# etri/bwa-mem-scale

Measured on AMD Instinct MI355X. Metric: Mreads/sec through the GPU hot path (seed -> chain -> extend -> dedup, reads and index resident), 150bp SE vs a synthetic genome of GRCh38 size, at 1 MI355X; % HBM roofline in roofline.frac, higher is better.
Workload: dtype int64 intervals / int16 DP (two columns per register; int32 for queries beyond 191 bases or scores beyond 2^14)

## Files before the change

bwa-mem-scale_amd/csrc/api.hip:

```cpp
#include <fcntl.h>
#include <sys/mman.h>
#include <sys/stat.h>
#include <unistd.h>

#include <algorithm>
#include <cstring>

#include "stage_state.h"

namespace bwams {

static Knobs g_knobs;
static std::once_flag g_knobs_once;
static int env_int(const char *name, int dflt) { const char *e = getenv(name); return e && *e ? atoi(e) : dflt; }
void knobs_reload() {
    Knobs k;
    { const char *vb = getenv("BWAMS_VERBOSE"); k.verbose = vb && *vb && *vb != '0'; }
    k.debug = env_int("BWAMS_DEBUG", 0);
    k.poison = env_int("BWAMS_POISON", 0);
    k.bwd_min_list = env_int("BWAMS_BWD_MIN_LIST", k.bwd_min_list); k.bwd_cols = env_int("BWAMS_BWD_COLS", k.bwd_cols);
    k.bwd_late_list = env_int("BWAMS_BWD_LATE_LIST", k.bwd_late_list);
    k.bwd_dry_min_list = env_int("BWAMS_BWD_DRY_MIN_LIST", k.bwd_dry_min_list); k.bwd_dry_cols = env_int("BWAMS_BWD_DRY_COLS", k.bwd_dry_cols);
    k.bwd_dry_late_list = env_int("BWAMS_BWD_DRY_LATE_LIST", k.bwd_dry_late_list);
    k.r3_beside = env_int("BWAMS_SEED_R3_BESIDE", 1);
    k.ext_max_rounds = env_int("BWAMS_EXT_MAX_ROUNDS", 0); k.ext_all_rounds = getenv("BWAMS_EXT_ALL_ROUNDS") != nullptr;
    k.ext_inplace = env_int("BWAMS_EXT_INPLACE", 1);
    k.dedup_seq = env_int("BWAMS_DEDUP_SEQ", 0) == 1;
    k.dedup_count = env_int("BWAMS_DEDUP_COUNT", 0) == 1;
    k.pair_count = env_int("BWAMS_PAIR_COUNT", 0) == 1;
    k.pair_drop_plan = getenv("BWAMS_PAIR_DROP_PLAN") != nullptr;
    k.trace_pair = env_int("BWAMS_TRACE_PAIR", 0);
    k.bsw_pk = env_int("BWAMS_BSW_PK", 1);
    k.chain_batch = env_int("BWAMS_CHAIN_BATCH", 1);
    k.chain_count = env_int("BWAMS_CHAIN_COUNT", 0) == 1;
    k.depth_combine = env_int("BWAMS_DEPTH_COMBINE", 1);
    k.pileup_tiled = env_int("BWAMS_PILEUP_TILED", 1);
    k.qc_lanes = env_int("BWAMS_QC_LANES", 1);
    k.recal_lds = env_int("BWAMS_RECAL_LDS", 1);
    k.ert_ticket = env_int("BWAMS_ERT_TICKET", 1); k.ert_grid = env_int("BWAMS_ERT_GRID", -1); k.ert_fat = env_int("BWAMS_ERT_FAT", 1);
    k.sa_dense = env_int("BWAMS_SA_DENSE", kSaDenseDefault);
    if (k.sa_dense != 0 && k.sa_dense != 1 && k.sa_dense != 2 && k.sa_dense != 4) k.sa_dense = kSaDenseDefault;
    { const char *mb = getenv("BWAMS_SA_DENSE_MAX_BYTES"); k.sa_dense_max_bytes = mb && *mb ? atoll(mb) : 0; }
    k.sort_narrow = env_int("BWAMS_SORT_NARROW", 1);
    g_knobs = k;
}
const Knobs &knobs() {
    std::call_once(g_knobs_once, knobs_reload);
    return g_knobs;
}

static thread_local std::string g_last_error;
void set_last_error(const std::string &s) { g_last_error = s; }

int check_device(int device) {
    int n = 0;
// ... 208 lines not shown
```

bwa-mem-scale_amd/csrc/api_extend.hip:

```cpp
#include <cstddef>

#include "stage_state.h"

using namespace bwams;

extern "C" {
static int ext_args(bwams_batch *b, StageState *s, const bwams_mem_opt_t *opt, ExtArgs *A) {
    const int64_t n1 = s->ch.nseq + 1;
    A->chains = s->ch.chains.p; A->n_chains = s->ch.n_chains; A->seeds = s->ch.seeds.p; A->n_seeds = s->ch.n_seeds;
    A->chain_off = s->ch.chain_off.as<int64_t>(); A->seed_off = s->ch.chain_off.as<int64_t>() + n1; A->enc = b->d_enc.p; A->cum = b->d_cum.p;
    A->nseq = s->ch.nseq; A->ref = b->idx->fmi.ref;
    int rc = dev_bns(b->idx, &A->bns);
    if (rc) return rc;
    A->opt = *opt; A->regs = s->ext.regs.p; A->srt = s->ext.srt.p; A->rmax = s->ext.rmax.as<int64_t>(); A->cnt = s->ext.cnt.as<int32_t>();
    A->ctr = b->d_ctr.p; A->state = s->ext.state.p; A->kreg = s->ext.kreg.p; A->cur = s->ext.cur.p; A->lim = s->ext.lim.p; A->sel_heavy = s->heavy.p;
    A->n_sel_heavy = &b->d_ctr.p->sel_heavy; A->sel_ticket = b->d_ctr.p->ext_sel_ticket; A->req_list = s->ext.req_list.p; A->rtask = nullptr;
    return BWAMS_OK;
}

static hipError_t ext_round_clear(bwams_batch *b) {
    DevCounters *c = b->d_ctr.p;
    return hipMemsetAsync(&c->ext_n_req, 0, (size_t)((char *)(c->ext_n_retry + 2) - (char *)&c->ext_n_req), b->stream);
}
static int ext_round_fetch(bwams_batch *b, int64_t *n_req, int64_t *n_rest, int64_t *n_l, int64_t *n_r) {
// ... 100 lines not shown
    if (n_right) *n_right = tot[3];
    produced(b, Product::built);
    return BWAMS_OK;
}

static int run_side(bwams_batch *b, StageState *s, const ExtArgs &A, int right, int64_t *n_retry_out) {
    hipStream_t st = b->stream;
    bwams_seqpair_t *pairs = right ? s->ext.rpairs.p : s->ext.lpairs.p;
    const bool ip = s->ext.tasks_inplace;
    const uint8_t *ref = ip ? A.ref : (right ? s->ext.rref.p : s->ext.lref.p);
    const uint8_t *qer = ip ? A.enc : (right ? s->ext.rqer.p : s->ext.lqer.p);
    const int64_t *src = ip ? (right ? s->ext.rsrc.as<int64_t>() : s->ext.lsrc.as<int64_t>()) : nullptr;
    const int dir = ip && !right ? -1 : 1;
    const int64_t n = right ? s->ext.n_right : s->ext.n_left;
    SwParams prm;
    sw_params(A.opt, right ? A.opt.pen_clip3 : A.opt.pen_clip5, &prm);
    const int qmax = b->max_read_len > 1 ? b->max_read_len : 1;
    if (n == 0) return BWAMS_OK;
    unsigned long long *d_nretry = &b->d_ctr.p->ext_n_retry[right], *h_nretry = &b->h_ctr.p->ext_n_retry[right];
    bwams_seqpair_t *rp = A.rtask ? s->ext.rpairs.p : nullptr;
    if (bsw_list_bytes(n) > b->sw.d_bsw_list.cap) BWAMS_HIP(hipStreamSynchronize(st));
    BWAMS_HIP(b->sw.d_bsw_list.ensure(bsw_list_bytes(n), bsw_list_bytes(n + n / 4 + 1024)));
    const bool verbose_bsw = knobs().verbose != 0;
    if (verbose_bsw) BWAMS_HIP(hipMemsetAsync(b->d_ctr.p->dbg + 40, 0, 8 * sizeof(unsigned long long), st));
    if (int lrc = launch_bsw(pairs, n, ref, qer, A.opt.w, prm, qmax, b->d_ctr.p, b->cu_count, st, b->sw.d_bsw_list.p, s->aux, s->fork, s->join, src, dir)) {
        set_last_error(lrc == -2 ? "banded SW: a query longer than ~18000 bases does not fit the LDS kernel" : "banded SW: stream fork/join failed");
        return lrc == -2 ? BWAMS_ERR_UNSUPPORTED : BWAMS_ERR_DEVICE;
    }
    launch_ext_post(A, right, pairs, n, A.opt.w, 0, s->ext.retry.p, d_nretry, rp, st);
    BWAMS_HIP(hipMemcpyAsync(h_nretry, d_nretry, sizeof(unsigned long long), hipMemcpyDeviceToHost, st));
    BWAMS_HIP(hipStreamSynchronize(st));
    if (verbose_bsw) {
        unsigned long long d[8];
        BWAMS_HIP(hipMemcpy(d, b->d_ctr.p->dbg + 40, sizeof d, hipMemcpyDeviceToHost));
        if (d[6])
            fprintf(stderr, "[run_side] bsw_pk_kernel, %s, %lld tasks: %llu waves, Mticks of wave-time %.2f, in the refill branch %.2f (%.1f %%), in the pass %.2f; "
                            "%llu refill events, %llu slots filled, %llu iterations\n",
                    right ? "right" : "left", (long long)n, d[6], d[0] / 1e6, d[1] / 1e6, 100. * (double)d[1] / (double)d[0], d[2] / 1e6, d[3], d[4], d[5]);
    }
    const unsigned long long nr = *h_nretry;
    if (nr) {
        if (launch_bsw(s->ext.retry.p, (int64_t)nr, ref, qer, A.opt.w << 1, prm, qmax, b->d_ctr.p, b->cu_count, st, b->sw.d_bsw_list.p, s->aux, s->fork, s->join, src, dir)) return BWAMS_ERR_DEVICE;
        launch_ext_post(A, right, s->ext.retry.p, (int64_t)nr, A.opt.w << 1, 1, nullptr, d_nretry, rp, st);
    }
    *n_retry_out += (int64_t)nr;
    return BWAMS_OK;
}

int bwams_extend_run(bwams_batch_t *b, const bwams_mem_opt_t *opt, int64_t *n_regs) {
    if (!has(b, Product::chains)) {
        set_last_error("bwams_extend_run: run bwams_chain_run (or bwams_chain_upload) first");
        return BWAMS_ERR_ARG;
    }
    if (!b->idx->fmi.ref) {
        set_last_error("bwams_extend_run: the index was opened without its .0123 reference");
        return BWAMS_ERR_ARG;
    }
    int rc = check_opt(opt, "bwams_extend_run");
    if (rc) return rc;
    int kMaxRounds = 6;
    if (knobs().ext_max_rounds > 0) kMaxRounds = knobs().ext_max_rounds;
    const bool adaptive_off = knobs().ext_all_rounds != 0;
    const bool inplace_on = knobs().ext_inplace != 0;
    StageState *s = b->stages;
    BWAMS_HIP(hipSetDevice(b->idx->device));
// ... 103 lines not shown
```

bwa-mem-scale_amd/csrc/api_sw.hip:

```cpp
#include "stage_state.h"

using namespace bwams;

extern "C" {

int bwams_bsw_upload(bwams_batch_t *b, const bwams_seqpair_t *pairs, int64_t n, const uint8_t *ref,
                     int64_t ref_bytes, const uint8_t *qer, int64_t qer_bytes) {
    if (!b || n < 0 || (n && (!pairs || !ref || !qer))) return BWAMS_ERR_ARG;
    BWAMS_HIP(hipSetDevice(b->idx->device));
    int qmax = 1, tmax = 1;
    for (int64_t i = 0; i < n; ++i) {
        const bwams_seqpair_t &p = pairs[i];
        if (p.len1 < 0 || p.len2 < 0 || p.idr < 0 || p.idq < 0 || (int64_t)p.idr + p.len1 > ref_bytes ||
            (int64_t)p.idq + p.len2 > qer_bytes) {
            set_last_error("bwams_bsw_upload: pair " + std::to_string(i) + " points outside the sequence buffers");
            return BWAMS_ERR_ARG;
        }
        if (p.len2 > qmax) qmax = p.len2;
        if (p.len1 > tmax) tmax = p.len1;
    }
    if (bsw_lds_waves(qmax) < 1) {
        set_last_error("bwams_bsw_upload: query of " + std::to_string(qmax) + " bases, longer than the LDS-resident kernel supports (18196)");
        return BWAMS_ERR_UNSUPPORTED;
    }
// ... 7 lines not shown
        BWAMS_HIP(hipMemcpyAsync(b->sw.d_qer.p, qer, (size_t)qer_bytes, hipMemcpyHostToDevice, b->stream));
        BWAMS_HIP(hipStreamSynchronize(b->stream));
    }
    b->sw.n_pairs = n;
    b->sw.max_qlen = qmax;
    b->sw.max_tlen = tmax;
    return BWAMS_OK;
}

int bwams_bsw_run(bwams_batch_t *b, int32_t w, const bwams_sw_opt_t *o) {
    if (!b || !o) return BWAMS_ERR_ARG;
    if (o->e_ins <= 0 || o->e_del <= 0) {
        set_last_error("bwams_bsw_run: gap extension penalties must be positive");
        return BWAMS_ERR_ARG;
    }
    BWAMS_HIP(hipSetDevice(b->idx->device));
    SwParams prm;
    sw_params(*o, &prm);
    BWAMS_HIP(hipMemsetAsync(&b->d_ctr.p->bsw_cells, 0, sizeof(unsigned long long), b->stream));
    const size_t list_bytes = b->sw.n_pairs > 0 ? bsw_list_bytes(b->sw.n_pairs) : 0;
    if (list_bytes > b->sw.d_bsw_list.cap) BWAMS_HIP(hipStreamSynchronize(b->stream));
    BWAMS_HIP(b->sw.d_bsw_list.ensure(list_bytes, bsw_list_bytes(b->sw.n_pairs + b->sw.n_pairs / 4 + 1024)));
    BWAMS_HIP(hipEventRecord(b->ev[b->kEvBswStart], b->stream));
    if (launch_bsw(b->sw.d_pairs.p, b->sw.n_pairs, b->sw.d_ref.p, b->sw.d_qer.p, w, prm, b->sw.max_qlen, b->d_ctr.p, b->cu_count, b->stream, b->sw.d_bsw_list.p)) {
        set_last_error("bwams_bsw_run: a query longer than ~18000 bases does not fit the LDS kernel");
        return BWAMS_ERR_UNSUPPORTED;
    }
    BWAMS_HIP(hipEventRecord(b->ev[b->kEvBswEnd], b->stream));
    BWAMS_HIP(hipGetLastError());
    return BWAMS_OK;
}

int bwams_bsw_fetch(bwams_batch_t *b, bwams_seqpair_t *pairs, int64_t n) {
    if (!b || n != b->sw.n_pairs) return BWAMS_ERR_ARG;
    BWAMS_HIP(hipSetDevice(b->idx->device));
    if (n) BWAMS_HIP(hipMemcpyAsync(pairs, b->sw.d_pairs.p, (size_t)n * sizeof(bwams_seqpair_t), hipMemcpyDeviceToHost, b->stream));
    BWAMS_HIP(hipStreamSynchronize(b->stream));
    return BWAMS_OK;
}

int bwams_bsw_extend(bwams_batch_t *b, bwams_seqpair_t *pairs, int64_t n, const uint8_t *ref, int64_t ref_bytes,
                     const uint8_t *qer, int64_t qer_bytes, int32_t w, const bwams_sw_opt_t *opt) {
    int rc = bwams_bsw_upload(b, pairs, n, ref, ref_bytes, qer, qer_bytes);
    if (rc) return rc;
    rc = bwams_bsw_run(b, w, opt);
    if (rc) return rc;
    return bwams_bsw_fetch(b, pairs, n);
// ... 42 lines not shown
```

bwa-mem-scale_amd/csrc/bsw_extend.hip:

```cpp
#include "common.h"
#include "wave_ops.h"

namespace bwams {

namespace {

constexpr int kWavesPerBlock = 4;
constexpr int kTaskChunk = 8;
constexpr size_t kBswLdsMax = 160 * 1024;

__host__ __device__ __forceinline__ size_t bsw_row_bytes(int qmax) {
    return (((size_t)(qmax + 1) * 8 + (size_t)qmax + 64 + 15) / 16) * 16;
}

__device__ __forceinline__ int wave_incl_prefix_max(int v, int lane) {
#pragma unroll
    for (int o = 1; o < 64; o <<= 1) {
        const int t = __shfl_up(v, o);
        if (lane >= o) v = max(v, t);
    }
    return v;
}

__global__ __launch_bounds__(kWavesPerBlock * 64) void bsw_kernel(
// ... 464 lines not shown
                ++i;
                fin = i >= tlen;
            }
            if (fin) {
                if (g == 0) {
                    bwams_seqpair_t *o = &pairs[cur];
                    o->score = mx; o->qle = max_j + 1; o->tle = max_i + 1; o->gtle = max_ie + 1; o->gscore = gscore; o->max_off = max_off;
                }
                alive = false;
            }
        }
    }
    for (int o = 32; o > 0; o >>= 1) cells += ((unsigned long long)__shfl_down((unsigned)(cells >> 32), o) << 32) | (unsigned)__shfl_down((unsigned)cells, o);
    if (lane == 0 && cells) atomicAdd(&ctr->bsw_cells, cells);
}


namespace pk {
__device__ __forceinline__ uint32_t add(uint32_t a, uint32_t b) { uint32_t d; asm("v_pk_add_u16 %0, %1, %2" : "=v"(d) : "v"(a), "v"(b)); return d; }
__device__ __forceinline__ uint32_t sub(uint32_t a, uint32_t b) { uint32_t d; asm("v_pk_sub_i16 %0, %1, %2" : "=v"(d) : "v"(a), "v"(b)); return d; }
__device__ __forceinline__ uint32_t max(uint32_t a, uint32_t b) { uint32_t d; asm("v_pk_max_i16 %0, %1, %2" : "=v"(d) : "v"(a), "v"(b)); return d; }
__device__ __forceinline__ uint32_t max0(uint32_t a) { uint32_t d; asm("v_pk_max_i16 %0, %1, 0" : "=v"(d) : "v"(a)); return d; }
__device__ __forceinline__ uint32_t mul(uint32_t a, uint32_t b) { uint32_t d; asm("v_pk_mul_lo_u16 %0, %1, %2" : "=v"(d) : "v"(a), "v"(b)); return d; }
__device__ __forceinline__ uint32_t adds(uint32_t a, uint32_t s) { uint32_t d; asm("v_pk_add_u16 %0, %1, %2" : "=v"(d) : "v"(a), "s"(s)); return d; }
__device__ __forceinline__ uint32_t subs(uint32_t a, uint32_t s) { uint32_t d; asm("v_pk_sub_i16 %0, %1, %2" : "=v"(d) : "v"(a), "s"(s)); return d; }
__device__ __forceinline__ uint32_t add2(uint32_t a) { uint32_t d; asm("v_pk_add_u16 %0, %1, 2 op_sel_hi:[1,0]" : "=v"(d) : "v"(a)); return d; }
__device__ __forceinline__ uint32_t min1(uint32_t a) { uint32_t d; asm("v_pk_min_u16 %0, %1, 1 op_sel_hi:[1,0]" : "=v"(d) : "v"(a)); return d; }
__device__ __forceinline__ uint32_t hi2(uint32_t a) { return __builtin_amdgcn_perm(a, a, 0x03020302u); }
__device__ __forceinline__ uint32_t lo2(uint32_t a) { return __builtin_amdgcn_perm(a, a, 0x01000100u); }
__device__ __forceinline__ uint32_t bfi(uint32_t mask, uint32_t a, uint32_t b) { uint32_t d; asm("v_bfi_b32 %0, %1, %2, %3" : "=v"(d) : "v"(mask), "v"(a), "v"(b)); return d; }
template <int CTRL> __device__ __forceinline__ int qdpp(int v) { return __builtin_amdgcn_update_dpp(0, v, CTRL, 0xF, 0xF, true); }
__device__ __forceinline__ int quad_all_max(int v) {
    int t = qdpp<0xB1>(v);
    v = v > t ? v : t;
    t = qdpp<0x4E>(v);
    return v > t ? v : t;
}
}

constexpr int kPkNeg = -16384;
#ifndef BWAMS_PK_WAVES
#define BWAMS_PK_WAVES 2
#endif
constexpr int kPkWaves = BWAMS_PK_WAVES;

__host__ __device__ __forceinline__ bool bsw_pk_eligible(const SwParams &prm) {
    for (int i = 0; i < 5; ++i)
        if (prm.mat[i * 5 + 4] != -1 || prm.mat[4 * 5 + i] != -1) return false;
    return prm.e_ins >= 0 && prm.e_ins <= 64 && prm.e_del >= 0 && prm.e_del <= 64 && prm.o_ins >= 0 && prm.o_ins + prm.e_ins < 8000 &&
           prm.o_del >= 0 && prm.o_del + prm.e_del < 8000;
}

__global__ __launch_bounds__(kPkWaves * 64) void bsw_pk_kernel(
    bwams_seqpair_t *__restrict__ pairs, const int32_t *__restrict__ list, const unsigned long long *n_list_p,
    const uint8_t *__restrict__ ref, const uint8_t *__restrict__ qer, int w0, SwParams prm, DevCounters *ctr, unsigned long long *head,
    int cols, const int64_t *__restrict__ src, int dir) {
    extern __shared__ __align__(16) uint32_t pk_lds[];
    constexpr int LPT = 4, TPW = 16;
    const int lane = threadIdx.x & 63, g = lane & (LPT - 1), q = lane / LPT;
    const int P = cols >> 1;
    uint32_t *const t_hp = pk_lds + 16 + (size_t)((threadIdx.x >> 6) * TPW + q) * (size_t)((5 * P) / 2 + 6);
    uint32_t *const t_ep = t_hp + P + 2;
    uint16_t *const t_sel = reinterpret_cast<uint16_t *>(t_ep + P + 2);
    uint16_t *const t_hp16 = reinterpret_cast<uint16_t *>(t_hp), *const t_ep16 = reinterpret_cast<uint16_t *>(t_ep);
    const int o_del = prm.o_del, e_del = prm.e_del, o_ins = prm.o_ins, e_ins = prm.e_ins;
    const int oe_del = o_del + e_del, oe_ins = o_ins + e_ins;
    uint2 *const pk_tab16 = reinterpret_cast<uint2 *>(pk_lds);
    if (threadIdx.x < 5) {
        const int t = threadIdx.x;
        pk_tab16[t] = make_uint2((uint32_t)(uint16_t)(int16_t)prm.mat[t * 5 + 0] | ((uint32_t)(uint16_t)(int16_t)prm.mat[t * 5 + 1] << 16),
                                 (uint32_t)(uint16_t)(int16_t)prm.mat[t * 5 + 2] | ((uint32_t)(uint16_t)(int16_t)prm.mat[t * 5 + 3] << 16));
    }
    __syncthreads();
    const uint32_t OEI = (uint32_t)oe_ins * 0x10001u, OED = (uint32_t)oe_del * 0x10001u, EDX = (uint32_t)e_del * 0x10001u;
    const uint32_t E1X = (uint32_t)e_ins * 0x10001u, E2X = (uint32_t)(2 * e_ins) * 0x10001u;
    const uint32_t NEGP = (uint32_t)(uint16_t)(int16_t)kPkNeg * 0x10001u;
    const int64_t n_list = (int64_t)*n_list_p;
    const unsigned long long kLeaders = 0x1111111111111111ull;
    int64_t pid = 0, pid_end = 0;
    bool exhausted = false;
    bool alive = false;
    int64_t pid0 = 0, s_qo = 0, s_to = 0;
    int s_cur = 0, s_tlen = 0, s_w = 0;
    uint32_t s_qh = 0u;
    int cur = 0, qlen = 0, tlen = 0, h0 = 0, w = 0, i = 0, beg = 0, end = 0;
    int mx = 0, max_i = -1, max_j = -1, max_ie = -1, gscore = -1, max_off = 0, tb_next = 4;
    const uint8_t *tr = ref;
    unsigned long long cells = 0;
    bool start_row = true, row = false;
    int base = 0, h1 = 0, key = -1, hlast = -1, c_max = kPkNeg, c_h = 0;
    int nz_last = 0, nz_first = 256;
    uint2 tt = make_uint2(0u, 0u);
#ifdef BWAMS_BSWDBG
    const unsigned long long T0 = __builtin_amdgcn_s_memtime();
    unsigned long long t_refill = 0, t_pass = 0, n_events = 0, n_filled = 0, n_iter = 0;
#endif

    for (;;) {
        const unsigned long long need_m = __ballot(!alive);
        if (need_m) {
#ifdef BWAMS_BSWDBG
            const unsigned long long Ta = __builtin_amdgcn_s_memtime();
#endif
            if (pid >= pid_end && !exhausted) {
                pid = (int64_t)wave_ticket(head, (unsigned long long)kQuadChunk);
                pid_end = pid + kQuadChunk < n_list ? pid + kQuadChunk : n_list;
                if (pid >= n_list) { exhausted = true; pid_end = pid; }
                pid0 = pid;
                if (lane < kQuadChunk && pid + lane < pid_end) {
                    s_cur = list[pid + lane];
                    const bwams_seqpair_t *sp = &pairs[s_cur];
                    const int l2 = sp->len2, hh0 = sp->h0;
                    s_tlen = sp->len1;
                    if (src) { const int64_t id = sp->id; s_qo = src[2 * id]; s_to = src[2 * id + 1]; }
                    else { s_qo = (int64_t)sp->idq; s_to = (int64_t)sp->idr; }
                    uint32_t tb = s_tlen > 0 ? (uint32_t)ref[s_to] : 4u;
                    tb = tb > 4u ? 4u : tb;
                    s_qh = (uint32_t)l2 | ((uint32_t)hh0 << 8) | (tb << 24);
// ... 1 lines not shown
                    int max_ins = (int)((double)(l2 * prm.max_sc + prm.end_bonus - o_ins) / e_ins + 1.);
                    max_ins = max_ins > 1 ? max_ins : 1;
                    ww = ww < max_ins ? ww : max_ins;
                    int max_del = (int)((double)(l2 * prm.max_sc + prm.end_bonus - o_del) / e_del + 1.);
                    max_del = max_del > 1 ? max_del : 1;
                    s_w = ww < max_del ? ww : max_del;
                }
            }
            const int avail = (int)(pid_end - pid);
            const int nq = __popcll(need_m & kLeaders);
            const int rank = __popcll(need_m & kLeaders & ((1ull << (q * LPT)) - 1ull));
            if (avail > 0) {
                const bool take = !alive && rank < avail;
                const int sk = take ? (int)(pid - pid0) + rank : 0;
                const int f_cur = __shfl(s_cur, sk), f_tlen = __shfl(s_tlen, sk), f_w = __shfl(s_w, sk);
                const uint32_t f_qh = (uint32_t)__shfl((int)s_qh, sk);
                const int64_t f_qo = shfl64(s_qo, sk), f_to = shfl64(s_to, sk);
                if (take) {
                    cur = f_cur; qlen = (int)(f_qh & 0xffu); h0 = (int)((f_qh >> 8) & 0x3fffu); tlen = f_tlen; w = f_w;
                    tr = ref + f_to;
                    start_row = true;
                    mx = h0; max_i = -1; max_j = -1; max_ie = -1; gscore = -1; max_off = 0;
                    beg = 0; end = qlen; i = 0;
                    alive = tlen > 0;
                    if (!alive && g == 0) {
                        bwams_seqpair_t *o = &pairs[cur];
                        o->score = mx; o->qle = 0; o->tle = 0; o->gtle = 0; o->gscore = -1; o->max_off = 0;
                    }
                    tb_next = (int)(f_qh >> 24);
                }
                for (unsigned long long fill_m = __ballot(take) & kLeaders; fill_m; fill_m &= fill_m - 1ull) {
                    const int sl = __ffsll((long long)fill_m) - 1;
                    const int f_qlen = __builtin_amdgcn_readlane(qlen, sl), f_h0 = __builtin_amdgcn_readlane(h0, sl);
                    const uint8_t *const f_q = qer + readlane64(f_qo, sl);
                    uint32_t *const f_hp = pk_lds + 16 + (size_t)((threadIdx.x >> 6) * TPW + (sl >> 2)) * (size_t)((5 * P) / 2 + 6);
                    uint32_t *const f_ep = f_hp + P + 2;
                    uint16_t *const f_sel = reinterpret_cast<uint16_t *>(f_ep + P + 2);
                    const int c0 = 4 * lane, p_last = f_qlen >> 1;
                    const bool full = c0 + 3 < f_qlen, edge = !full && c0 < f_qlen;
                    uint32_t v = 0u, b0 = 4u, b1 = 4u, b2 = 4u;
                    if (full) __builtin_memcpy(&v, dir > 0 ? f_q + c0 : f_q - c0 - 3, 4);
                    if (edge) {
                        const int last = f_qlen - 1;
                        b0 = f_q[c0 * dir];
                        b1 = f_q[(c0 + 1 < last ? c0 + 1 : last) * dir];
                        b2 = f_q[(c0 + 2 < last ? c0 + 2 : last) * dir];
// ... 31 lines not shown
            if (exhausted && !wave_any(alive)) break;
        }
#ifdef BWAMS_BSWDBG
        const unsigned long long Tb = __builtin_amdgcn_s_memtime();
#endif

        asm volatile("; BSW_PK_PASS_BEGIN");
        if (alive && start_row) {
            int tb = tb_next;
            tb = tb > 4 ? 4 : tb;
            if (i + 1 < tlen) tb_next = tr[(i + 1) * dir];
            tt = pk_tab16[tb];
            if (beg < i - w) beg = i - w;
            if (end > i + w + 1) end = i + w + 1;
            if (end > qlen) end = qlen;
            h1 = 0;
            if (beg == 0) {
                h1 = h0 - (o_del + e_del * (i + 1));
                h1 = h1 < 0 ? 0 : h1;
            }
            row = beg < end;
            key = -1; hlast = -1; nz_last = 0; nz_first = 256;
            c_max = kPkNeg; c_h = 0;
            base = beg & ~3;
            start_row = false;
        }
        {
            const bool in = alive && row;
            const int jb = base + g * 8;
            const bool inr = in && jb < cols;
            int lo = beg - jb, hi = end - jb;
            lo = lo < 0 ? 0 : (lo > 8 ? 8 : lo);
            hi = hi < 0 ? 0 : (hi > 8 ? 8 : hi);
            const uint32_t m8 = inr ? ((1u << hi) - 1u) & ~((1u << lo) - 1u) : 0u;
            const uint32_t m8x = m8 | (m8 << 15);
            const int pj = inr ? (jb >> 1) : 0;
            const uint2 hpa = *reinterpret_cast<const uint2 *>(t_hp + pj), hpb = *reinterpret_cast<const uint2 *>(t_hp + pj + 2);
            const uint2 epa = *reinterpret_cast<const uint2 *>(t_ep + pj), epb = *reinterpret_cast<const uint2 *>(t_ep + pj + 2);
            uint2 sl2;
            sl2.x = *reinterpret_cast<const uint32_t *>(t_sel + pj);
            sl2.y = *reinterpret_cast<const uint32_t *>(t_sel + pj + 2);
            const uint32_t hpv[4] = {hpa.x, hpa.y, hpb.x, hpb.y}, epv[4] = {epa.x, epa.y, epb.x, epb.y};
            const uint32_t slv[4] = {__builtin_amdgcn_perm(sl2.x, sl2.x, 0x01010000u) + 0x01000100u, __builtin_amdgcn_perm(sl2.x, sl2.x, 0x03030202u) + 0x01000100u,
                                     __builtin_amdgcn_perm(sl2.y, sl2.y, 0x01010000u) + 0x01000100u, __builtin_amdgcn_perm(sl2.y, sl2.y, 0x03030202u) + 0x01000100u};
            uint32_t AM[4], M[4], E[4], PX[4], JE[4], JP[4];
            JE[0] = (uint32_t)(jb * e_ins) * 0x10001u + ((uint32_t)e_ins << 16);
// ... 42 lines not shown
            for (int c = 0; c < 4; ++c) { F4[c] = pk::max(F4[c], Lexp); E2[c] = pk::subs(M[c], OED); }
#pragma unroll
            for (int c = 0; c < 4; ++c) { F4[c] = pk::sub(F4[c], JE[c]); T1[c] = pk::subs(E[c], EDX); ME[c] = pk::max(M[c], E[c]); }
#pragma unroll
            for (int c = 0; c < 4; ++c) { F4[c] = pk::adds(F4[c], E1X); E2[c] = pk::max(E2[c], T1[c]); }
#pragma unroll
            for (int c = 0; c < 4; ++c) { F4[c] = pk::max0(F4[c]); E2[c] = pk::max0(E2[c]); }
#pragma unroll
            for (int c = 0; c < 4; ++c) Hn[c] = pk::max(ME[c], F4[c]);
            const int h3 = (int)(Hn[3] >> 16);
            int hin = pk::qdpp<0x90>(h3);
            hin = g == 0 ? c_h : hin;
            uint32_t HL[4];
            HL[0] = __builtin_amdgcn_alignbit(Hn[0], (uint32_t)hin << 16, 16);
#pragma unroll
            for (int c = 1; c < 4; ++c) HL[c] = __builtin_amdgcn_alignbit(Hn[c], Hn[c - 1], 16);
            if (m8) {
                *reinterpret_cast<uint2 *>(t_hp + pj) = make_uint2(pk::bfi(AM[0], HL[0], hpv[0]), pk::bfi(AM[1], HL[1], hpv[1]));
                *reinterpret_cast<uint2 *>(t_hp + pj + 2) = make_uint2(pk::bfi(AM[2], HL[2], hpv[2]), pk::bfi(AM[3], HL[3], hpv[3]));
                *reinterpret_cast<uint2 *>(t_ep + pj) = make_uint2(pk::bfi(AM[0], E2[0], epv[0]), pk::bfi(AM[1], E2[1], epv[1]));
                *reinterpret_cast<uint2 *>(t_ep + pj + 2) = make_uint2(pk::bfi(AM[2], E2[2], epv[2]), pk::bfi(AM[3], E2[3], epv[3]));
            }
            int lkey = -1;
#pragma unroll
            for (int c = 0; c < 4; ++c) {
                const uint32_t ha = Hn[c] & AM[c];
                const int k0 = (int)__builtin_amdgcn_perm(ha, JP[c], 0x0c050400u), k1 = (int)__builtin_amdgcn_perm(ha, JP[c], 0x0c070602u);
                const int kk = k0 > k1 ? k0 : k1;
                lkey = lkey > kk ? lkey : kk;
            }
            {
                uint32_t NF[4];
#pragma unroll
                for (int c = 0; c < 4; ++c) NF[c] = (HL[c] | E2[c]) & AM[c];
#pragma unroll
                for (int c = 0; c < 4; ++c) NF[c] = pk::min1(NF[c]);
                const uint32_t nx = NF[0] | (NF[1] << 2) | (NF[2] << 4) | (NF[3] << 6);
                const int nl = (int)(((nx | (nx >> 15)) & 0xffu) << (8 * g));
                int nw = nl | pk::qdpp<0xB1>(nl);
                nw |= pk::qdpp<0x4E>(nw);
                const bool any = nw != 0;
                const int fc = any ? base + __builtin_ctz((unsigned)nw) : 256;
                nz_last = any ? base + 32 - __builtin_clz((unsigned)nw) : nz_last;
                nz_first = nz_first < fc ? nz_first : fc;
            }
            lkey = m8 ? lkey : -1;
            key = key > lkey ? key : lkey;
            {
                const int oe = hi - 1;
                if (m8 && jb + hi == end) {
                    uint32_t hv = Hn[0];
                    hv = (oe >> 1) == 1 ? Hn[1] : hv;
                    hv = (oe >> 1) == 2 ? Hn[2] : hv;
                    hv = (oe >> 1) == 3 ? Hn[3] : hv;
                    hlast = (int)((hv >> ((oe & 1) << 4)) & 0xffffu);
                }
            }
            if (in && base == (beg & ~3) && h1 != 0 && g == 0) t_hp16[beg] = (uint16_t)h1;
            const int pm = pk::qdpp<0xFF>(scan);
            const int ch = pk::qdpp<0xFF>(h3);
            const bool more = in && base + LPT * 8 < end;
            if (more) {
                c_max = c_max > pm ? c_max : pm;
                c_h = ch;
                base += LPT * 8;
            }
            const int rkey = pk::quad_all_max(key), rhl = pk::quad_all_max(hlast);
            int last_nz = nz_last - 1;
            int first_nz = nz_first;
            if (alive && !more) {
                if (row && h1 != 0) {
                    first_nz = first_nz < beg ? first_nz : beg;
                    last_nz = last_nz > beg ? last_nz : beg;
                }
                const int m = row ? rkey >> 8 : 0, mj = row ? (rkey & 0xff) - 1 : -1;
                const int h1f = row ? rhl : h1;
                if (g == 0) { t_hp16[end] = (uint16_t)h1f; t_ep16[end] = 0; }
                if (row) cells += (unsigned long long)(g == 0 ? end - beg : 0);
                const int j_exit = row ? end : beg;
                if (j_exit == qlen) {
                    max_ie = gscore > h1f ? max_ie : i;
                    gscore = gscore > h1f ? gscore : h1f;
                }
                const bool better = m > mx;
                const int di = i - max_i, dj = mj - max_j;
                const int zpen = di > dj ? (di - dj) * e_del : (dj - di) * e_ins;
                bool fin = m == 0 || (!better && prm.zdrop > 0 && mx - m - zpen > prm.zdrop);
                {
                    int d = mj - i;
                    d = d < 0 ? -d : d;
                    d = max_off > d ? max_off : d;
                    max_off = better ? d : max_off;
                    max_i = better ? i : max_i;
                    max_j = better ? mj : max_j;
                    mx = better ? m : mx;
                }
                {
                    const int nbeg = first_nz < end ? first_nz : end;
                    int jj = last_nz >= nbeg ? last_nz : nbeg - 1;
                    jj = h1f != 0 ? end : jj;
                    beg = nbeg;
                    end = jj + 2 < qlen ? jj + 2 : qlen;
                    ++i;
                    fin = fin || i >= tlen;
                }
                if (fin) {
                    if (g == 0) {
                        bwams_seqpair_t *o = &pairs[cur];
                        o->score = mx; o->qle = max_j + 1; o->tle = max_i + 1; o->gtle = max_ie + 1; o->gscore = gscore; o->max_off = max_off;
                    }
                    alive = false;
                }
                start_row = true;
            }
        }
        asm volatile("; BSW_PK_PASS_END");
#ifdef BWAMS_BSWDBG
        asm volatile("s_waitcnt vmcnt(0) lgkmcnt(0)" ::: "memory");
        t_pass += __builtin_amdgcn_s_memtime() - Tb;
        ++n_iter;
#endif
    }
#ifdef BWAMS_BSWDBG
    if (lane == 0) {
        unsigned long long *d = ctr->dbg + 40;
        atomicAdd(&d[0], __builtin_amdgcn_s_memtime() - T0); atomicAdd(&d[1], t_refill); atomicAdd(&d[2], t_pass);
        atomicAdd(&d[3], n_events); atomicAdd(&d[4], n_filled); atomicAdd(&d[5], n_iter); atomicAdd(&d[6], 1ull);
    }
#endif
    for (int o = 32; o > 0; o >>= 1) cells += ((unsigned long long)__shfl_down((unsigned)(cells >> 32), o) << 32) | (unsigned)__shfl_down((unsigned)cells, o);
    if (lane == 0 && cells) atomicAdd(&ctr->bsw_cells, cells);
}

__global__ void bsw_reset_kernel(DevCounters *ctr) {
    for (int i = 0; i < 4; ++i) ctr->bsw_head[i] = 0;
    for (int i = 0; i < kNumBswClass; ++i) ctr->bsw_cls_cnt[i] = ctr->bsw_cls_head[i] = 0;
}

}

int launch_bsw(bwams_seqpair_t *pairs, int64_t n, const uint8_t *ref, const uint8_t *qer, int w, const SwParams &prm, int qmax,
               DevCounters *ctr, int cu_count, hipStream_t st, int32_t *list, hipStream_t *aux, hipEvent_t fork, hipEvent_t *join,
               const int64_t *src, int dir) {
    bsw_reset_kernel<<<1, 1, 0, st>>>(ctr);
    if (n <= 0) return 0;
    bsw_classify_kernel<<<(unsigned)((n + 1023) / 1024), 1024, 0, st>>>(pairs, n, prm.max_sc, list, ctr->bsw_cls_cnt);
    int64_t blocks = (n + kWavesPerBlock - 1) / kWavesPerBlock;
    const int64_t maxb = (int64_t)cu_count * 8;
    if (blocks > maxb) blocks = maxb;
    hipStream_t q[5] = {st, st, st, st, st};
    const int n_aux = aux ? 4 : 0;
    if (n_aux) {
        if (hipEventRecord(fork, st) != hipSuccess) return -1;
        for (int c = 0; c < n_aux; ++c) {
            q[c + 1] = aux[c];
            if (hipStreamWaitEvent(q[c + 1], fork, 0) != hipSuccess) return -1;
        }
    }
    const unsigned B = (unsigned)blocks, T = kWavesPerBlock * 64;
    unsigned long long *cnt = ctr->bsw_cls_cnt, *hd = ctr->bsw_cls_head;
    auto pk_lds = [](int cols) { return (size_t)64 + (size_t)kPkWaves * 16 * ((size_t)(cols / 2) * 10 + 24); };
    {
        static std::mutex mu;
        static bool done[64] = {};
        int dev = 0;
        if (hipGetDevice(&dev) != hipSuccess) return -1;
        std::lock_guard<std::mutex> g(mu);
        if (dev < 0 || dev >= 64 || !done[dev]) {
            if (hipFuncSetAttribute(reinterpret_cast<const void *>(bsw_qwin_kernel<kBswLpt, kBswWin>), hipFuncAttributeMaxDynamicSharedMemorySize,
                                    (int)((size_t)kWavesPerBlock * (64 / kBswLpt) * 192 * 4)) != hipSuccess) return -1;
            if (hipFuncSetAttribute(reinterpret_cast<const void *>(bsw_pk_kernel), hipFuncAttributeMaxDynamicSharedMemorySize, (int)pk_lds(192)) != hipSuccess) return -1;
            if (dev >= 0 && dev < 64) done[dev] = true;
        }
    }
    const bool pk_env = knobs().bsw_pk != 0;
    if (pk_env && bsw_pk_eligible(prm)) {
        static const int kCols[5] = {32, 64, 96, 144, 192};
        const unsigned Bp = (unsigned)((int64_t)B * kWavesPerBlock / kPkWaves);
        for (int c = 4; c >= 0; --c)
            bsw_pk_kernel<<<Bp, kPkWaves * 64, pk_lds(kCols[c]), q[c]>>>(pairs, list + (int64_t)c * n, cnt + c, ref, qer, w, prm, ctr, hd + c, kCols[c], src, dir);
    } else {
    bsw_qwin_kernel<kBswLpt, kBswWin><<<B, T, (size_t)kWavesPerBlock * (64 / kBswLpt) * 192 * 4, q[4]>>>(pairs, list + 4 * n, cnt + 4, ref, qer, w, prm, ctr, hd + 4, 192, src, dir);
    bsw_qwin_kernel<kBswLpt, kBswWin><<<B, T, (size_t)kWavesPerBlock * (64 / kBswLpt) * 144 * 4, q[3]>>>(pairs, list + 3 * n, cnt + 3, ref, qer, w, prm, ctr, hd + 3, 144, src, dir);
    bsw_qwin_kernel<kBswLpt, kBswWin><<<B, T, (size_t)kWavesPerBlock * (64 / kBswLpt) * 96 * 4, q[2]>>>(pairs, list + 2 * n, cnt + 2, ref, qer, w, prm, ctr, hd + 2, 96, src, dir);
    bsw_qwin_kernel<kBswLpt, kBswWin><<<B, T, (size_t)kWavesPerBlock * (64 / kBswLpt) * 64 * 4, q[1]>>>(pairs, list + 1 * n, cnt + 1, ref, qer, w, prm, ctr, hd + 1, 64, src, dir);
    bsw_qwin_kernel<kBswLpt, kBswWin><<<B, T, (size_t)kWavesPerBlock * (64 / kBswLpt) * 32 * 4, q[0]>>>(pairs, list + 0 * n, cnt + 0, ref, qer, w, prm, ctr, hd + 0, 32, src, dir);
    }
    {
        const int waves = bsw_lds_waves(qmax);
        if (waves < 1) return -2;
        const size_t lds = bsw_row_bytes(qmax) * (size_t)waves;
        if (lds > 48 * 1024)
            (void)hipFuncSetAttribute(reinterpret_cast<const void *>(bsw_kernel),
                                      hipFuncAttributeMaxDynamicSharedMemorySize, (int)lds);
        int64_t lblocks = (n + waves - 1) / waves;
        const int64_t lcap = qmax > 16 * kQuadCpl[4] - 1 ? maxb : (int64_t)cu_count * 2;
        if (lblocks > lcap) lblocks = lcap;
        bsw_kernel<<<(unsigned)lblocks, waves * 64, lds, q[0]>>>(pairs, n, ref, qer, w, prm, qmax, -1, ctr, &ctr->bsw_head[3], list + 5 * n, cnt + 5, src, dir);
    }
    if (n_aux)
        for (int c = 0; c < n_aux; ++c) {
            if (hipEventRecord(join[c], q[c + 1]) != hipSuccess) return -1;
            if (hipStreamWaitEvent(st, join[c], 0) != hipSuccess) return -1;
// ... 12 lines not shown
```

bwa-mem-scale_amd/csrc/common.h:

```cpp
#pragma once

#include <atomic>
#include <cstdlib>
#include <hip/hip_runtime.h>
#include <mutex>
#include <shared_mutex>
#include <stdint.h>
#include <stdio.h>
#include <string>
#include <vector>

#include "../../include/bwams.h"
#include "stage_valid.h"

namespace bwams {

void set_last_error(const std::string &s);

constexpr int kSaDenseDefault = 1;
struct Knobs {
    int verbose = 0;
    int debug = 0;
    int poison = 0;
    int bwd_min_list = 40, bwd_cols = 24, bwd_late_list = 8;
    int bwd_dry_min_list = 24, bwd_dry_cols = 8, bwd_dry_late_list = 12;
    int r3_beside = 1;
    int ext_max_rounds = 0;
    int ext_all_rounds = 0;
    int ext_inplace = 1;
    int dedup_seq = 0;
    int dedup_count = 0;
    int pair_count = 0;
    int pair_drop_plan = 0;
    int trace_pair = 0;
    int bsw_pk = 1;
    int chain_count = 0;
    int chain_batch = 1;
    int ert_fat = 1;
    int depth_combine = 1;
    int pileup_tiled = 1;
    int qc_lanes = 1;
    int recal_lds = 1;
    int ert_grid = -1, ert_ticket = 1;
    int sa_dense = kSaDenseDefault;
    int64_t sa_dense_max_bytes = 0;
    int sort_narrow = 1;
};
const Knobs &knobs();
void knobs_reload();

int sa_dense_release(int device);

template <class T> static inline hipError_t dev_malloc(T **p, size_t bytes, bool may_yield = true) {
    const bool poison = knobs().poison != 0;
    hipError_t e = hipMalloc(reinterpret_cast<void **>(p), bytes);
    if (e == hipErrorOutOfMemory && may_yield) {
        int dev = 0;
        (void)hipGetLastError();
// ... 637 lines not shown
                       int out_on_device, int32_t flags, int64_t *n_out, bwams_deflate_stats_t *stats);

struct SwParams {
    int o_del, e_del, o_ins, e_ins, zdrop, end_bonus, max_sc;
    int8_t mat[25];
};

struct Round2Work {
    uint32_t rid;
    int32_t x;
    int32_t min_intv;
};

struct BwdItem {
    uint32_t rid;
    int32_t x;
    int32_t min_intv;
    int32_t num_prev;
    int64_t off;
};

int launch_bsw(bwams_seqpair_t *pairs, int64_t n, const uint8_t *ref, const uint8_t *qer, int w, const SwParams &prm, int qmax,
               DevCounters *ctr, int cu_count, hipStream_t st, int32_t *list, hipStream_t *aux = nullptr, hipEvent_t fork = nullptr,
               hipEvent_t *join = nullptr, const int64_t *src = nullptr, int dir = 1);
size_t bsw_list_bytes(int64_t n_tasks);
int bsw_lds_waves(int qmax);
void launch_emf_probe(const DevEmf &t, const uint8_t *enc, const int64_t *cum, int64_t nseq, uint32_t *out,
                      uint8_t *code, uint8_t *skip, DevCounters *ctr, hipStream_t st);
constexpr int KSW_XBYTE = 0x10000, KSW_XSTOP = 0x20000, KSW_XSUBO = 0x40000, KSW_XSTART = 0x80000;
constexpr int kKswMaxTarget = 20000;
int launch_ksw(const bwams_seqpair_t *pairs, int64_t n, const uint8_t *ref, const uint8_t *qer, const SwParams &prm,
                int pmax, int tmax, void *out, DevCounters *ctr, int cu_count, hipStream_t st);

struct SegMove { const char *src; char *dst; int64_t len; };
int segment_copy(const std::vector<SegMove> &moves, hipStream_t st);
int line_ends(const char *d_text, int64_t n_bytes, hipStream_t st, DevBuf<int64_t> *ends, int64_t *n_nl);

struct BnsMeta {
    int64_t l_pac = 0;
    std::vector<std::string> names, comments;
    std::vector<int64_t> ctg_off;
    std::vector<int32_t> ctg_len, ctg_ambs;
    std::vector<int64_t> hole_off;
    std::vector<int32_t> hole_len;
    std::vector<char> hole_amb;
    DevBuf<> d_pac;
};
// ... 194 lines not shown
```

Measured before the change: 11.95.

## Add early-termination bound to packed banded SW extension kernel

Adds a templated early-exit path to the packed int16 banded Smith-Waterman kernel. Each row computes an upper bound on the score any remaining cell could still reach (per-cell H/E plus the remaining query times the match score, and h1 plus the full query score). Once the band's tail is known and that bound cannot beat the current max or the global score, the task stops. It is on by default in the extension path (knob default -1) and adds per-row packed arithmetic plus a cross-lane max. It also pins waves_per_eu to 4, which may change register allocation and occupancy.

```diff
diff --git a/bwa-mem-scale_amd/csrc/api.hip b/bwa-mem-scale_amd/csrc/api.hip
--- a/bwa-mem-scale_amd/csrc/api.hip
+++ b/bwa-mem-scale_amd/csrc/api.hip
@@ -31,6 +31,7 @@
     k.pair_drop_plan = getenv("BWAMS_PAIR_DROP_PLAN") != nullptr;
     k.trace_pair = env_int("BWAMS_TRACE_PAIR", 0);
     k.bsw_pk = env_int("BWAMS_BSW_PK", 1);
+    k.bsw_early = env_int("BWAMS_BSW_EARLY", -1);
     k.chain_batch = env_int("BWAMS_CHAIN_BATCH", 1);
     k.chain_count = env_int("BWAMS_CHAIN_COUNT", 0) == 1;
     k.depth_combine = env_int("BWAMS_DEPTH_COMBINE", 1);
diff --git a/bwa-mem-scale_amd/csrc/api_extend.hip b/bwa-mem-scale_amd/csrc/api_extend.hip
--- a/bwa-mem-scale_amd/csrc/api_extend.hip
+++ b/bwa-mem-scale_amd/csrc/api_extend.hip
@@ -146,8 +146,9 @@
     if (bsw_list_bytes(n) > b->sw.d_bsw_list.cap) BWAMS_HIP(hipStreamSynchronize(st));
     BWAMS_HIP(b->sw.d_bsw_list.ensure(bsw_list_bytes(n), bsw_list_bytes(n + n / 4 + 1024)));
     const bool verbose_bsw = knobs().verbose != 0;
-    if (verbose_bsw) BWAMS_HIP(hipMemsetAsync(b->d_ctr.p->dbg + 40, 0, 8 * sizeof(unsigned long long), st));
-    if (int lrc = launch_bsw(pairs, n, ref, qer, A.opt.w, prm, qmax, b->d_ctr.p, b->cu_count, st, b->sw.d_bsw_list.p, s->aux, s->fork, s->join, src, dir)) {
+    const bool early = knobs().bsw_early != 0;
+    if (verbose_bsw) BWAMS_HIP(hipMemsetAsync(b->d_ctr.p->dbg + 40, 0, 10 * sizeof(unsigned long long), st));
+    if (int lrc = launch_bsw(pairs, n, ref, qer, A.opt.w, prm, qmax, b->d_ctr.p, b->cu_count, st, b->sw.d_bsw_list.p, s->aux, s->fork, s->join, src, dir, early)) {
         set_last_error(lrc == -2 ? "banded SW: a query longer than ~18000 bases does not fit the LDS kernel" : "banded SW: stream fork/join failed");
         return lrc == -2 ? BWAMS_ERR_UNSUPPORTED : BWAMS_ERR_DEVICE;
     }
@@ -155,16 +156,16 @@
     BWAMS_HIP(hipMemcpyAsync(h_nretry, d_nretry, sizeof(unsigned long long), hipMemcpyDeviceToHost, st));
     BWAMS_HIP(hipStreamSynchronize(st));
     if (verbose_bsw) {
-        unsigned long long d[8];
+        unsigned long long d[10];
         BWAMS_HIP(hipMemcpy(d, b->d_ctr.p->dbg + 40, sizeof d, hipMemcpyDeviceToHost));
         if (d[6])
             fprintf(stderr, "[run_side] bsw_pk_kernel, %s, %lld tasks: %llu waves, Mticks of wave-time %.2f, in the refill branch %.2f (%.1f %%), in the pass %.2f; "
-                            "%llu refill events, %llu slots filled, %llu iterations\n",
-                    right ? "right" : "left", (long long)n, d[6], d[0] / 1e6, d[1] / 1e6, 100. * (double)d[1] / (double)d[0], d[2] / 1e6, d[3], d[4], d[5]);
+                            "%llu refill events, %llu slots filled, %llu iterations, %llu rows, %llu tasks ended early\n",
+                    right ? "right" : "left", (long long)n, d[6], d[0] / 1e6, d[1] / 1e6, 100. * (double)d[1] / (double)d[0], d[2] / 1e6, d[3], d[4], d[5], d[7], d[8]);
     }
     const unsigned long long nr = *h_nretry;
     if (nr) {
-        if (launch_bsw(s->ext.retry.p, (int64_t)nr, ref, qer, A.opt.w << 1, prm, qmax, b->d_ctr.p, b->cu_count, st, b->sw.d_bsw_list.p, s->aux, s->fork, s->join, src, dir)) return BWAMS_ERR_DEVICE;
+        if (launch_bsw(s->ext.retry.p, (int64_t)nr, ref, qer, A.opt.w << 1, prm, qmax, b->d_ctr.p, b->cu_count, st, b->sw.d_bsw_list.p, s->aux, s->fork, s->join, src, dir, early)) return BWAMS_ERR_DEVICE;
         launch_ext_post(A, right, s->ext.retry.p, (int64_t)nr, A.opt.w << 1, 1, nullptr, d_nretry, rp, st);
     }
     *n_retry_out += (int64_t)nr;
diff --git a/bwa-mem-scale_amd/csrc/api_sw.hip b/bwa-mem-scale_amd/csrc/api_sw.hip
--- a/bwa-mem-scale_amd/csrc/api_sw.hip
+++ b/bwa-mem-scale_amd/csrc/api_sw.hip
@@ -53,7 +53,8 @@
     if (list_bytes > b->sw.d_bsw_list.cap) BWAMS_HIP(hipStreamSynchronize(b->stream));
     BWAMS_HIP(b->sw.d_bsw_list.ensure(list_bytes, bsw_list_bytes(b->sw.n_pairs + b->sw.n_pairs / 4 + 1024)));
     BWAMS_HIP(hipEventRecord(b->ev[b->kEvBswStart], b->stream));
-    if (launch_bsw(b->sw.d_pairs.p, b->sw.n_pairs, b->sw.d_ref.p, b->sw.d_qer.p, w, prm, b->sw.max_qlen, b->d_ctr.p, b->cu_count, b->stream, b->sw.d_bsw_list.p)) {
+    if (launch_bsw(b->sw.d_pairs.p, b->sw.n_pairs, b->sw.d_ref.p, b->sw.d_qer.p, w, prm, b->sw.max_qlen, b->d_ctr.p, b->cu_count, b->stream, b->sw.d_bsw_list.p,
+                   nullptr, nullptr, nullptr, nullptr, 1, knobs().bsw_early == 1)) {
         set_last_error("bwams_bsw_run: a query longer than ~18000 bases does not fit the LDS kernel");
         return BWAMS_ERR_UNSUPPORTED;
     }
diff --git a/bwa-mem-scale_amd/csrc/bsw_extend.hip b/bwa-mem-scale_amd/csrc/bsw_extend.hip
--- a/bwa-mem-scale_amd/csrc/bsw_extend.hip
+++ b/bwa-mem-scale_amd/csrc/bsw_extend.hip
@@ -510,6 +510,7 @@
 __device__ __forceinline__ uint32_t max(uint32_t a, uint32_t b) { uint32_t d; asm("v_pk_max_i16 %0, %1, %2" : "=v"(d) : "v"(a), "v"(b)); return d; }
 __device__ __forceinline__ uint32_t max0(uint32_t a) { uint32_t d; asm("v_pk_max_i16 %0, %1, 0" : "=v"(d) : "v"(a)); return d; }
 __device__ __forceinline__ uint32_t mul(uint32_t a, uint32_t b) { uint32_t d; asm("v_pk_mul_lo_u16 %0, %1, %2" : "=v"(d) : "v"(a), "v"(b)); return d; }
+__device__ __forceinline__ uint32_t mad(uint32_t a, uint32_t b, uint32_t c) { uint32_t d; asm("v_pk_mad_u16 %0, %1, %2, %3" : "=v"(d) : "v"(a), "v"(b), "v"(c)); return d; }
 __device__ __forceinline__ uint32_t adds(uint32_t a, uint32_t s) { uint32_t d; asm("v_pk_add_u16 %0, %1, %2" : "=v"(d) : "v"(a), "s"(s)); return d; }
 __device__ __forceinline__ uint32_t subs(uint32_t a, uint32_t s) { uint32_t d; asm("v_pk_sub_i16 %0, %1, %2" : "=v"(d) : "v"(a), "s"(s)); return d; }
 __device__ __forceinline__ uint32_t add2(uint32_t a) { uint32_t d; asm("v_pk_add_u16 %0, %1, 2 op_sel_hi:[1,0]" : "=v"(d) : "v"(a)); return d; }
@@ -530,6 +531,10 @@
 #ifndef BWAMS_PK_WAVES
 #define BWAMS_PK_WAVES 2
 #endif
+#ifndef BWAMS_BSW_EARLY_FORM
+#define BWAMS_BSW_EARLY_FORM 1
+#endif
+constexpr int kPkEarlyForm = BWAMS_BSW_EARLY_FORM;
 constexpr int kPkWaves = BWAMS_PK_WAVES;
 
 __host__ __device__ __forceinline__ bool bsw_pk_eligible(const SwParams &prm) {
@@ -539,7 +544,8 @@
            prm.o_del >= 0 && prm.o_del + prm.e_del < 8000;
 }
 
-__global__ __launch_bounds__(kPkWaves * 64) void bsw_pk_kernel(
+template <int EARLY>
+__global__ __launch_bounds__(kPkWaves * 64) __attribute__((amdgpu_waves_per_eu(4, 4))) void bsw_pk_kernel(
     bwams_seqpair_t *__restrict__ pairs, const int32_t *__restrict__ list, const unsigned long long *n_list_p,
     const uint8_t *__restrict__ ref, const uint8_t *__restrict__ qer, int w0, SwParams prm, DevCounters *ctr, unsigned long long *head,
     int cols, const int64_t *__restrict__ src, int dir) {
@@ -579,9 +585,11 @@
     int base = 0, h1 = 0, key = -1, hlast = -1, c_max = kPkNeg, c_h = 0;
     int nz_last = 0, nz_first = 256;
     uint2 tt = make_uint2(0u, 0u);
+    int zr = 0;
+    uint32_t pot = 0u;
 #ifdef BWAMS_BSWDBG
     const unsigned long long T0 = __builtin_amdgcn_s_memtime();
-    unsigned long long t_refill = 0, t_pass = 0, n_events = 0, n_filled = 0, n_iter = 0;
+    unsigned long long t_refill = 0, t_pass = 0, n_events = 0, n_filled = 0, n_iter = 0, n_rows = 0, n_rule = 0;
 #endif
 
     for (;;) {
@@ -629,6 +637,7 @@
                     start_row = true;
                     mx = h0; max_i = -1; max_j = -1; max_ie = -1; gscore = -1; max_off = 0;
                     beg = 0; end = qlen; i = 0;
+                    if constexpr (EARLY != 0) zr = qlen;
                     alive = tlen > 0;
                     if (!alive && g == 0) {
                         bwams_seqpair_t *o = &pairs[cur];
@@ -706,6 +715,7 @@
             row = beg < end;
             key = -1; hlast = -1; nz_last = 0; nz_first = 256;
             c_max = kPkNeg; c_h = 0;
+            if constexpr (EARLY != 0) pot = 0u;
             base = beg & ~3;
             start_row = false;
         }
@@ -794,6 +804,20 @@
                 *reinterpret_cast<uint2 *>(t_ep + pj + 2) = make_uint2(pk::bfi(AM[2], E2[2], epv[2]), pk::bfi(AM[3], E2[3], epv[3]));
             }
             int lkey = -1;
+            if constexpr (EARLY != 0) {
+                const uint32_t A2X = (uint32_t)(2 * prm.max_sc) * 0x10001u;
+                uint32_t RM[4], X[4], T[4];
+                RM[0] = pk::lo2((uint32_t)__mul24(qlen - 1 - jb, prm.max_sc)) - ((uint32_t)prm.max_sc << 16);
+#pragma unroll
+                for (int c = 1; c < 4; ++c) RM[c] = pk::subs(RM[c - 1], A2X);
+#pragma unroll
+                for (int c = 0; c < 4; ++c) X[c] = pk::max(Hn[c] & AM[c], E2[c]);
+#pragma unroll
+                for (int c = 0; c < 4; ++c) T[c] = pk::min1(X[c]);
+#pragma unroll
+                for (int c = 0; c < 4; ++c) X[c] = pk::mad(T[c], RM[c], X[c]);
+                pot = pk::max(pot, pk::max(pk::max(X[0], X[1]), pk::max(X[2], X[3])));
+            }
 #pragma unroll
             for (int c = 0; c < 4; ++c) {
                 const uint32_t ha = Hn[c] & AM[c];
@@ -838,6 +862,11 @@
                 base += LPT * 8;
             }
             const int rkey = pk::quad_all_max(key), rhl = pk::quad_all_max(hlast);
+            int rpot = 0;
+            if constexpr (EARLY != 0) {
+                const int a = (int)(pot & 0xffffu), b = (int)(pot >> 16);
+                rpot = pk::quad_all_max(a > b ? a : b);
+            }
             int last_nz = nz_last - 1;
             int first_nz = nz_first;
             if (alive && !more) {
@@ -871,6 +900,21 @@
                     const int nbeg = first_nz < end ? first_nz : end;
                     int jj = last_nz >= nbeg ? last_nz : nbeg - 1;
                     jj = h1f != 0 ? end : jj;
+                    if constexpr (EARLY != 0) {
+                        int P = h1 + __mul24(qlen, prm.max_sc);
+                        P = h1 > 0 ? P : 0;
+                        P = P > rpot ? P : rpot;
+                        const bool tail_known = end >= zr;
+                        zr = tail_known ? jj : zr;
+                        const bool ends = tail_known && P <= mx && P < gscore && (EARLY == 1 || (i & 3) == 3);
+#ifdef BWAMS_BSWDBG
+                        if (g == 0 && ends && !fin && i + 1 < tlen) ++n_rule;
+#endif
+                        fin = fin || ends;
+                    }
+#ifdef BWAMS_BSWDBG
+                    if (g == 0) ++n_rows;
+#endif
                     beg = nbeg;
                     end = jj + 2 < qlen ? jj + 2 : qlen;
                     ++i;
@@ -899,6 +943,7 @@
         atomicAdd(&d[0], __builtin_amdgcn_s_memtime() - T0); atomicAdd(&d[1], t_refill); atomicAdd(&d[2], t_pass);
         atomicAdd(&d[3], n_events); atomicAdd(&d[4], n_filled); atomicAdd(&d[5], n_iter); atomicAdd(&d[6], 1ull);
     }
+    if (g == 0 && n_rows) { atomicAdd(&ctr->dbg[47], n_rows); atomicAdd(&ctr->dbg[48], n_rule); }
 #endif
     for (int o = 32; o > 0; o >>= 1) cells += ((unsigned long long)__shfl_down((unsigned)(cells >> 32), o) << 32) | (unsigned)__shfl_down((unsigned)cells, o);
     if (lane == 0 && cells) atomicAdd(&ctr->bsw_cells, cells);
@@ -913,7 +958,7 @@
 
 int launch_bsw(bwams_seqpair_t *pairs, int64_t n, const uint8_t *ref, const uint8_t *qer, int w, const SwParams &prm, int qmax,
                DevCounters *ctr, int cu_count, hipStream_t st, int32_t *list, hipStream_t *aux, hipEvent_t fork, hipEvent_t *join,
-               const int64_t *src, int dir) {
+               const int64_t *src, int dir, bool early) {
     bsw_reset_kernel<<<1, 1, 0, st>>>(ctr);
     if (n <= 0) return 0;
     bsw_classify_kernel<<<(unsigned)((n + 1023) / 1024), 1024, 0, st>>>(pairs, n, prm.max_sc, list, ctr->bsw_cls_cnt);
@@ -941,7 +986,8 @@
         if (dev < 0 || dev >= 64 || !done[dev]) {
             if (hipFuncSetAttribute(reinterpret_cast<const void *>(bsw_qwin_kernel<kBswLpt, kBswWin>), hipFuncAttributeMaxDynamicSharedMemorySize,
                                     (int)((size_t)kWavesPerBlock * (64 / kBswLpt) * 192 * 4)) != hipSuccess) return -1;
-            if (hipFuncSetAttribute(reinterpret_cast<const void *>(bsw_pk_kernel), hipFuncAttributeMaxDynamicSharedMemorySize, (int)pk_lds(192)) != hipSuccess) return -1;
+            if (hipFuncSetAttribute(reinterpret_cast<const void *>(bsw_pk_kernel<0>), hipFuncAttributeMaxDynamicSharedMemorySize, (int)pk_lds(192)) != hipSuccess) return -1;
+            if (hipFuncSetAttribute(reinterpret_cast<const void *>(bsw_pk_kernel<kPkEarlyForm>), hipFuncAttributeMaxDynamicSharedMemorySize, (int)pk_lds(192)) != hipSuccess) return -1;
             if (dev >= 0 && dev < 64) done[dev] = true;
         }
     }
@@ -949,8 +995,9 @@
     if (pk_env && bsw_pk_eligible(prm)) {
         static const int kCols[5] = {32, 64, 96, 144, 192};
         const unsigned Bp = (unsigned)((int64_t)B * kWavesPerBlock / kPkWaves);
+        auto *const kern = early && prm.max_sc > 0 ? bsw_pk_kernel<kPkEarlyForm> : bsw_pk_kernel<0>;
         for (int c = 4; c >= 0; --c)
-            bsw_pk_kernel<<<Bp, kPkWaves * 64, pk_lds(kCols[c]), q[c]>>>(pairs, list + (int64_t)c * n, cnt + c, ref, qer, w, prm, ctr, hd + c, kCols[c], src, dir);
+            kern<<<Bp, kPkWaves * 64, pk_lds(kCols[c]), q[c]>>>(pairs, list + (int64_t)c * n, cnt + c, ref, qer, w, prm, ctr, hd + c, kCols[c], src, dir);
     } else {
     bsw_qwin_kernel<kBswLpt, kBswWin><<<B, T, (size_t)kWavesPerBlock * (64 / kBswLpt) * 192 * 4, q[4]>>>(pairs, list + 4 * n, cnt + 4, ref, qer, w, prm, ctr, hd + 4, 192, src, dir);
     bsw_qwin_kernel<kBswLpt, kBswWin><<<B, T, (size_t)kWavesPerBlock * (64 / kBswLpt) * 144 * 4, q[3]>>>(pairs, list + 3 * n, cnt + 3, ref, qer, w, prm, ctr, hd + 3, 144, src, dir);
diff --git a/bwa-mem-scale_amd/csrc/common.h b/bwa-mem-scale_amd/csrc/common.h
--- a/bwa-mem-scale_amd/csrc/common.h
+++ b/bwa-mem-scale_amd/csrc/common.h
@@ -34,6 +34,7 @@
     int pair_drop_plan = 0;
     int trace_pair = 0;
     int bsw_pk = 1;
+    int bsw_early = -1;
     int chain_count = 0;
     int chain_batch = 1;
     int ert_fat = 1;
@@ -717,7 +718,7 @@
 
 int launch_bsw(bwams_seqpair_t *pairs, int64_t n, const uint8_t *ref, const uint8_t *qer, int w, const SwParams &prm, int qmax,
                DevCounters *ctr, int cu_count, hipStream_t st, int32_t *list, hipStream_t *aux = nullptr, hipEvent_t fork = nullptr,
-               hipEvent_t *join = nullptr, const int64_t *src = nullptr, int dir = 1);
+               hipEvent_t *join = nullptr, const int64_t *src = nullptr, int dir = 1, bool early = false);
 size_t bsw_list_bytes(int64_t n_tasks);
 int bsw_lds_waves(int qmax);
 void launch_emf_probe(const DevEmf &t, const uint8_t *enc, const int64_t *cum, int64_t nseq, uint32_t *out,
```

Measured after the change: 12.38, median of 6. +3.5%, better.
